# arpitbansal297/Cold-Diffusion-Models

Hardware: NVIDIA H100
Metric: training-step images/sec (CelebA-128 deblur UNet, config 3) (higher is better)
Workload: dtype tf32

## Files before the change

### cold_diffusion_models_b200/csrc/conv_tc.cu

```cuda
#include "tc_common.cuh"
#include "conv_epilogue.cuh"

namespace {

constexpr int kTileM = 128;
constexpr int kChunkK = 32;
constexpr int kABytes = kTileM * 128;
constexpr int kThreads = 288;
constexpr int kConsumerWarps = 8;

struct TcParams {
  int B, Hg, Wg;
  int TW, TH, TN;
  int tiles_x, tiles_y, tiles_n, tiles_co, total_tiles;
  int sy, sx;
  int Cout;
  int nsrc;
  int ntaps[2];
  int kchunks[2];
  int wpb[2];
  int8_t dy[2][CD_MAX_TAPS];
  int8_t dx[2][CD_MAX_TAPS];
  float* out; int out_ld; int Ho, Wo; int oys, oxs, oy0, ox0;
  const float* bias;
  const float* resid; int resid_ld;
  int act; int round_tf32;
  float* out2; int out2_ld;
  const float* aux; int aux_ld;
  int nbox[2];
  int8_t boxdx[2][3];
  int8_t boxend[2][3];
  int8_t taporder[2][CD_MAX_TAPS];
  int tapoff[2][CD_MAX_TAPS];
};

__device__ __forceinline__ long long tile_pixel(const TcParams& p, int tile, int m) {
  int mt = tile / p.tiles_co;
  const int tx = mt % p.tiles_x; mt /= p.tiles_x;
  const int ty = mt % p.tiles_y;
  const int tn = mt / p.tiles_y;
  const int gx = tx * p.TW + m % p.TW, gy = ty * p.TH + (m / p.TW) % p.TH, b = tn * p.TN + m / (p.TW * p.TH);
  if (b >= p.B) return -1;
  return (static_cast<long long>(b) * p.Ho + (gy * p.oys + p.oy0)) * p.Wo + (gx * p.oxs + p.ox0);
}

__device__ __forceinline__ void epi_pair(const TcParams& p, long long pix, int col, float v0, float v1) {
  if (col + 1 < p.Cout) {
    float2 v = make_float2(v0, v1);
    if (p.bias) { const float2 b = __ldg(reinterpret_cast<const float2*>(p.bias + col)); v.x += b.x; v.y += b.y; }
    if (p.resid) { const float2 r = *reinterpret_cast<const float2*>(p.resid + pix * p.resid_ld + col); v.x += r.x; v.y += r.y; }
    if (p.out2) *reinterpret_cast<float2*>(p.out2 + pix * p.out2_ld + col) = v;
    if (p.act == CD_ACT_GELU) { v.x = cd_gelu(v.x); v.y = cd_gelu(v.y); }
    else if (p.act == CD_ACT_GELU_BWD) {
      const float2 a = *reinterpret_cast<const float2*>(p.aux + pix * p.aux_ld + col);
      v.x *= cd_gelu_grad(a.x); v.y *= cd_gelu_grad(a.y);
    }
    if (p.round_tf32) { v.x = cd_round_tf32(v.x); v.y = cd_round_tf32(v.y); }
    *reinterpret_cast<float2*>(p.out + pix * p.out_ld + col) = v;
  } else if (col < p.Cout) {
    float v = v0;
    if (p.bias) v += p.bias[col];
    if (p.resid) v += p.resid[pix * p.resid_ld + col];
    if (p.out2) p.out2[pix * p.out2_ld + col] = v;
    if (p.act == CD_ACT_GELU) v = cd_gelu(v);
    else if (p.act == CD_ACT_GELU_BWD) v *= cd_gelu_grad(p.aux[pix * p.aux_ld + col]);
    if (p.round_tf32) v = cd_round_tf32(v);
    p.out[pix * p.out_ld + col] = v;
  }
}

template <int BN, int STAGES, bool STG = false, bool F16 = false, int CTAS = 1, bool PAIR = false>
__global__ void __launch_bounds__(kThreads, CTAS)
conv_tc_kernel(const __grid_constant__ CUtensorMap mapA0, const __grid_constant__ CUtensorMap mapA1,
               const __grid_constant__ CUtensorMap mapB0, const __grid_constant__ CUtensorMap mapB1,
               const TcParams p) {
  constexpr int kBBytes = BN * 128;
  constexpr int kStageBytes = kABytes + kBBytes;
  constexpr int kChunkElems = F16 ? 64 : kChunkK;

  extern __shared__ uint8_t smem_raw[];
  const uint32_t raw_addr = smem_u32(smem_raw);
  const uint32_t pad = (1024u - (raw_addr & 1023u)) & 1023u;
  uint8_t* smem = smem_raw + pad;
  uint64_t* bars = reinterpret_cast<uint64_t*>(smem + STAGES * kStageBytes);
  uint64_t* full_bar = bars;
  uint64_t* empty_bar = bars + STAGES;
  static_assert(2 * STAGES * 8 <= 256, "barrier block is 256 bytes");
  float* epi_stage = reinterpret_cast<float*>(smem + STAGES * kStageBytes + 256);

  const int warp = threadIdx.x >> 5;
  const int lane = threadIdx.x & 31;
  const int wg = threadIdx.x >> 7;

  if (threadIdx.x == 0) {
    for (int i = 0; i < STAGES; ++i) { mbar_init(&full_bar[i], 1); mbar_init(&empty_bar[i], kConsumerWarps * (PAIR ? 2 : 1)); }
    asm volatile("fence.mbarrier_init.release.cluster;" ::: "memory");
  }
  if constexpr (PAIR) cluster_sync(); else __syncthreads();
  const uint32_t rank = PAIR ? cluster_ctarank() : 0;
  const int unit0 = PAIR ? blockIdx.x / 2 : blockIdx.x, ustride = PAIR ? gridDim.x / 2 : gridDim.x;
  const int units = PAIR ? p.tiles_co * ((p.total_tiles / p.tiles_co + 1) / 2) : p.total_tiles;
  auto tile_of = [&](int u) { return PAIR ? ((u / p.tiles_co) * 2 + static_cast<int>(rank)) * p.tiles_co + u % p.tiles_co : u; };

  const int kiters = p.ntaps[0] * p.kchunks[0] + (p.nsrc > 1 ? p.ntaps[1] * p.kchunks[1] : 0);

  if (warp == kConsumerWarps) {
    if (elect_one()) {
      uint32_t stage = 0, ph = 0;
      for (int u = unit0; u < units; u += ustride) {
        const int tile = tile_of(u);
        const int co_t = tile % p.tiles_co;
        int mt = tile / p.tiles_co;
        const int tx = mt % p.tiles_x; mt /= p.tiles_x;
        const int ty = mt % p.tiles_y;
        const int tn = mt / p.tiles_y;
        const int x0 = tx * p.TW * p.sx, y0 = ty * p.TH * p.sy, n0 = tn * p.TN, co0 = co_t * BN;
        for (int s = 0; s < p.nsrc; ++s) {
          const CUtensorMap* mA = s ? &mapA1 : &mapA0;
          const CUtensorMap* mB = s ? &mapB1 : &mapB0;
          const int wbase = p.wpb[s] ? n0 * p.ntaps[s] : 0;
          for (int tap = 0; tap < p.ntaps[s]; ++tap) {
            const int xin = x0 + p.dx[s][tap], yin = y0 + p.dy[s][tap];
            for (int kc = 0; kc < p.kchunks[s]; ++kc) {
              mbar_wait(&empty_bar[stage], ph ^ 1u);
              mbar_expect_tx(&full_bar[stage], kStageBytes);
              const uint32_t sa = smem_u32(smem + stage * kStageBytes);
              tma_load_4d(sa, mA, &full_bar[stage], kc * kChunkElems, xin, yin, n0);
              if constexpr (PAIR)
                tma_load_3d_mc(sa + kABytes + rank * (kBBytes / 2), mB, &full_bar[stage], kc * kChunkElems, co0 + static_cast<int>(rank) * (BN / 2),
                               wbase + tap, static_cast<uint16_t>(3));
              else
                tma_load_3d(sa + kABytes, mB, &full_bar[stage], kc * kChunkElems, co0, wbase + tap);
              if (++stage == STAGES) { stage = 0; ph ^= 1u; }
            }
          }
        }
      }
    }
    __syncwarp();
  } else {
    const int cw = wg;
    const int tid = threadIdx.x & 127;
    const int rl = (tid >> 5) * 16 + (lane >> 2);
    const int q2 = (lane & 3) * 2;
    float acc[BN / 2];
    uint32_t stage = 0, ph = 0;
    auto release = [&](uint32_t st) {
      __syncwarp();
      if (lane == 0) { mbar_arrive(&empty_bar[st]); if constexpr (PAIR) mbar_arrive_cluster(&empty_bar[st], rank ^ 1u); }
    };
    for (int u = unit0; u < units; u += ustride) {
      const int tile = tile_of(u);
      uint32_t prev = 0;
      for (int k = 0; k < kiters; ++k) {
        mbar_wait(&full_bar[stage], ph);
        wgmma_fence();
        const uint32_t sa = smem_u32(smem + stage * kStageBytes);
        const uint64_t da = make_kmajor_sw128_desc(sa + cw * (kABytes / 2));
        const uint64_t db = make_kmajor_sw128_desc(sa + kABytes);
#pragma unroll
        for (int kk = 0; kk < 4; ++kk) {
          if constexpr (F16) wgmma_f16<BN>(acc, da + uint64_t(kk * 2), db + uint64_t(kk * 2), (k | kk) != 0 ? 1u : 0u);
          else wgmma_tf32<BN>(acc, da + uint64_t(kk * 2), db + uint64_t(kk * 2), (k | kk) != 0 ? 1u : 0u);
        }
        wgmma_commit();
        wgmma_wait<1>();
        if (k > 0) release(prev);
        prev = stage;
        if (++stage == STAGES) { stage = 0; ph ^= 1u; }
      }
      wgmma_wait<0>();
      if (kiters > 0) release(prev);

      const int co0 = (tile % p.tiles_co) * BN;
      const long long pix0 = tile_pixel(p, tile, cw * 64 + rl);
      const long long pix1 = tile_pixel(p, tile, cw * 64 + rl + 8);
      if constexpr (STG) {
        float* st = epi_stage + cw * 64 * kEpiStageStride;
        const int bar_id = 1 + cw;
#pragma unroll
        for (int c = 0; c < BN; c += 32) {
          if (co0 + c + 32 <= p.Cout) {
            asm volatile("bar.sync %0, 128;" :: "r"(bar_id) : "memory");
#pragma unroll
            for (int j = c / 8; j < c / 8 + 4; ++j) {
              *reinterpret_cast<float2*>(st + rl * kEpiStageStride + 8 * j - c + q2) = make_float2(acc[4 * j], acc[4 * j + 1]);
              *reinterpret_cast<float2*>(st + (rl + 8) * kEpiStageStride + 8 * j - c + q2) = make_float2(acc[4 * j + 2], acc[4 * j + 3]);
            }
            asm volatile("bar.sync %0, 128;" :: "r"(bar_id) : "memory");
            const int w4 = tid >> 5;
            if (w4 < 2) {
              const int row = w4 * 32 + lane;
              uint32_t r[32];
#pragma unroll
              for (int e = 0; e < 32; ++e) r[e] = __float_as_uint(st[row * kEpiStageStride + e]);
              const long long pix = tile_pixel(p, tile, cw * 64 + row);
              cd_epilogue_staged32(r, st + w4 * 32 * kEpiStageStride, lane, pix < 0 ? 0 : pix, pix >= 0, co0 + c, p);
            }
          } else {
#pragma unroll
            for (int j = c / 8; j < c / 8 + 4; ++j) {
              if (pix0 >= 0) epi_pair(p, pix0, co0 + 8 * j + q2, acc[4 * j], acc[4 * j + 1]);
              if (pix1 >= 0) epi_pair(p, pix1, co0 + 8 * j + q2, acc[4 * j + 2], acc[4 * j + 3]);
            }
          }
        }
      } else {
#pragma unroll
        for (int j = 0; j < BN / 8; ++j) {
          if (pix0 >= 0) epi_pair(p, pix0, co0 + 8 * j + q2, acc[4 * j], acc[4 * j + 1]);
          if (pix1 >= 0) epi_pair(p, pix1, co0 + 8 * j + q2, acc[4 * j + 2], acc[4 * j + 3]);
        }
      }
    }
  }
  if constexpr (PAIR) cluster_sync();
}

constexpr int kRowsTW = 16, kRowsTH = kTileM / kRowsTW;
constexpr int kRowsBoxBytes = kRowsTW * (kRowsTH + 2) * 128;

template <int BN, int TH, int ABOXES, int STAGES>
__device__ __forceinline__ void rows_producer(const CUtensorMap& mapA0, const CUtensorMap& mapA1, const CUtensorMap& mapB0,
                                              const CUtensorMap& mapB1, const TcParams& p, uint8_t* abox, uint8_t* wtile,
                                              uint64_t* afull, uint64_t* aempty, uint64_t* full_bar, uint64_t* empty_bar) {
  constexpr int kBBytes = BN * 128;
  constexpr int kBoxBytes = kRowsTW * (TH + 2) * 128;
  if (elect_one()) {
    uint32_t stage = 0, ph = 0, ai = 0, aph = 0;
    for (int tile = blockIdx.x; tile < p.total_tiles; tile += gridDim.x) {
      const int co0 = (tile % p.tiles_co) * BN;
      int mt = tile / p.tiles_co;
      const int x0 = (mt % p.tiles_x) * kRowsTW; mt /= p.tiles_x;
      const int y0 = (mt % p.tiles_y) * TH;
      const int n = mt / p.tiles_y;
      for (int s = 0; s < p.nsrc; ++s) {
        const CUtensorMap* mA = s ? &mapA1 : &mapA0;
        const CUtensorMap* mB = s ? &mapB1 : &mapB0;
        for (int kc = 0; kc < p.kchunks[s]; ++kc) {
          for (int b = 0, i = 0; b < p.nbox[s]; ++b) {
            mbar_wait(&aempty[ai], aph ^ 1u);
            mbar_expect_tx(&afull[ai], kBoxBytes);
            tma_load_4d(smem_u32(abox + ai * kBoxBytes), mA, &afull[ai], kc * kChunkK, x0 + p.boxdx[s][b], y0 - 1, n);
            if (++ai == ABOXES) { ai = 0; aph ^= 1u; }
            for (; i < p.boxend[s][b]; ++i) {
              mbar_wait(&empty_bar[stage], ph ^ 1u);
              mbar_expect_tx(&full_bar[stage], kBBytes);
              tma_load_3d(smem_u32(wtile + stage * kBBytes), mB, &full_bar[stage], kc * kChunkK, co0, p.taporder[s][i]);
              if (++stage == STAGES) { stage = 0; ph ^= 1u; }
            }
          }
        }
      }
    }
  }
  __syncwarp();
}

template <int BN, int ABOXES, int STAGES, int CTAS>
__global__ void __launch_bounds__(kThreads, CTAS)
conv_rows_kernel(const __grid_constant__ CUtensorMap mapA0, const __grid_constant__ CUtensorMap mapA1,
                 const __grid_constant__ CUtensorMap mapB0, const __grid_constant__ CUtensorMap mapB1, const __grid_constant__ TcParams p) {
  constexpr int kBBytes = BN * 128;
  extern __shared__ uint8_t smem_raw[];
  const uint32_t raw_addr = smem_u32(smem_raw);
  uint8_t* smem = smem_raw + ((1024u - (raw_addr & 1023u)) & 1023u);
  uint8_t* abox = smem;
  uint8_t* wtile = smem + ABOXES * kRowsBoxBytes;
  uint64_t* bars = reinterpret_cast<uint64_t*>(wtile + STAGES * kBBytes);
  uint64_t* full_bar = bars;
  uint64_t* empty_bar = bars + STAGES;
  uint64_t* afull = bars + 2 * STAGES;
  uint64_t* aempty = bars + 2 * STAGES + ABOXES;
  static_assert(2 * (STAGES + ABOXES) * 8 <= 256, "barrier block is 256 bytes");
  const int warp = threadIdx.x >> 5, lane = threadIdx.x & 31, wg = threadIdx.x >> 7;
  if (threadIdx.x == 0) {
    for (int i = 0; i < STAGES; ++i) { mbar_init(&full_bar[i], 1); mbar_init(&empty_bar[i], kConsumerWarps); }
    for (int i = 0; i < ABOXES; ++i) { mbar_init(&afull[i], 1); mbar_init(&aempty[i], kConsumerWarps); }
    asm volatile("fence.mbarrier_init.release.cluster;" ::: "memory");
  }
  __syncthreads();

  if (warp == kConsumerWarps) {
    rows_producer<BN, kRowsTH, ABOXES, STAGES>(mapA0, mapA1, mapB0, mapB1, p, abox, wtile, afull, aempty, full_bar, empty_bar);
    return;
  }

  const int tid = threadIdx.x & 127;
  const int rl = (tid >> 5) * 16 + (lane >> 2);
  const int q2 = (lane & 3) * 2;
  auto release = [&](uint64_t* bar) { __syncwarp(); if (lane == 0) mbar_arrive(bar); };
  float acc[BN / 2];
  uint32_t stage = 0, ph = 0, ai = 0, aph = 0;
  for (int tile = blockIdx.x; tile < p.total_tiles; tile += gridDim.x) {
    int k = 0;
    uint32_t prev = 0, prev_a = 0;
    for (int s = 0; s < p.nsrc; ++s) {
      for (int kc = 0; kc < p.kchunks[s]; ++kc) {
        for (int b = 0, i = 0; b < p.nbox[s]; ++b) {
          mbar_wait(&afull[ai], aph);
          const uint32_t abase = smem_u32(abox + ai * kRowsBoxBytes) + wg * (kABytes / 2);
          for (const int i0 = i; i < p.boxend[s][b]; ++i, ++k) {
            mbar_wait(&full_bar[stage], ph);
            wgmma_fence();
            const uint64_t da = make_kmajor_sw128_desc(abase + p.tapoff[s][i]);
            const uint64_t db = make_kmajor_sw128_desc(smem_u32(wtile + stage * kBBytes));
#pragma unroll
            for (int kk = 0; kk < 4; ++kk)
              wgmma_tf32<BN>(acc, da + uint64_t(kk * 2), db + uint64_t(kk * 2), (k | kk) != 0 ? 1u : 0u);
            wgmma_commit();
            wgmma_wait<1>();
            if (k > 0) release(&empty_bar[prev]);
            if (k > 0 && i == i0) release(&aempty[prev_a]);
            prev = stage;
            if (++stage == STAGES) { stage = 0; ph ^= 1u; }
          }
          prev_a = ai;
          if (++ai == ABOXES) { ai = 0; aph ^= 1u; }
        }
      }
    }
    wgmma_wait<0>();
    if (k > 0) { release(&empty_bar[prev]); release(&aempty[prev_a]); }

    const int co0 = (tile % p.tiles_co) * BN;
    int mt = tile / p.tiles_co;
    const int x0 = (mt % p.tiles_x) * kRowsTW; mt /= p.tiles_x;
    const int y0 = (mt % p.tiles_y) * kRowsTH;
    const int n = mt / p.tiles_y;
#pragma unroll
    for (int h = 0; h < 2; ++h) {
      const int m = wg * 64 + rl + 8 * h;
      const int gx = x0 + m % kRowsTW, gy = y0 + m / kRowsTW;
      if (gx >= p.Wg || gy >= p.Hg) continue;
      const long long pix = (static_cast<long long>(n) * p.Ho + (gy * p.oys + p.oy0)) * p.Wo + (gx * p.oxs + p.ox0);
#pragma unroll
      for (int j = 0; j < BN / 8; ++j) epi_pair(p, pix, co0 + 8 * j + q2, acc[4 * j + 2 * h], acc[4 * j + 2 * h + 1]);
    }
  }
}

constexpr int kR256TH = 16;
constexpr int kR256BoxBytes = kRowsTW * (kR256TH + 2) * 128;
constexpr int kR256Slice = 128 * 128;
constexpr int kR256Threads = 384;
constexpr int kR256RegsLow = 40, kR256RegsHigh = 232;

constexpr int kOpFull = 0, kOpEmpty = 2, kBiasFull = 4, kBiasEmpty = 5, kEpiBars = 6;

__host__ __device__ __forceinline__ const float* rows256_operand(const TcParams& p) {
  return p.resid ? p.resid : (p.act == CD_ACT_GELU_BWD ? p.aux : nullptr);
}

template <int BN>
__device__ __forceinline__ void rows256_epilogue_producer(const CUtensorMap& mapE, const TcParams& p, int cw, uint8_t* so2,
                                                          float* sbias, uint64_t* eb) {
  const int lane = threadIdx.x & 31;
  const bool opnd = rows256_operand(p) != nullptr;
  uint32_t bph = 0, oph = 0;
  for (int tile = blockIdx.x; tile < p.total_tiles; tile += gridDim.x) {
    const int co0 = (tile % p.tiles_co) * BN;
    int mt = tile / p.tiles_co;
    const int x0 = (mt % p.tiles_x) * kRowsTW; mt /= p.tiles_x;
    const int yw = (mt % p.tiles_y) * kR256TH + 8 * cw;
    const int n = mt / p.tiles_y;
    if (yw >= p.Hg) continue;
    if (p.bias) {
      mbar_wait(&eb[kBiasEmpty], bph ^ 1u);
      for (int i = lane; i < BN; i += 32) sbias[i] = co0 + i < p.Cout ? p.bias[co0 + i] : 0.f;
      mbar_arrive(&eb[kBiasFull]);
      bph ^= 1u;
    }
    if (opnd && lane == 0) {
      for (int c = 0; c < BN / 32 && co0 + 32 * c < p.Cout; ++c)
        for (int h = 0; h < 2; ++h) {
          mbar_wait(&eb[kOpEmpty + h], ((oph >> h) & 1u) ^ 1u);
          mbar_expect_tx(&eb[kOpFull + h], kR256Slice / 2);
          tma_load_4d(smem_u32(so2 + h * (kR256Slice / 2)), &mapE, &eb[kOpFull + h], co0 + 32 * c, x0, yw + 4 * h, n);
          oph ^= 1u << h;
        }
    }
    __syncwarp();
  }
}

template <int BN, int ABOXES, int STAGES>
__global__ void __launch_bounds__(kR256Threads, 1)
conv_rows256_kernel(const __grid_constant__ CUtensorMap mapA0, const __grid_constant__ CUtensorMap mapA1,
                    const __grid_constant__ CUtensorMap mapB0, const __grid_constant__ CUtensorMap mapB1,
                    const __grid_constant__ CUtensorMap mapO, const __grid_constant__ CUtensorMap mapO2,
                    const __grid_constant__ CUtensorMap mapE, const __grid_constant__ TcParams p) {
  constexpr int kBBytes = BN * 128;
  extern __shared__ uint8_t smem_raw[];
  const uint32_t raw_addr = smem_u32(smem_raw);
  uint8_t* smem = smem_raw + ((1024u - (raw_addr & 1023u)) & 1023u);
  uint8_t* abox = smem;
  uint8_t* wtile = smem + ABOXES * kR256BoxBytes;
  uint8_t* stg = wtile + STAGES * kBBytes;
  uint64_t* bars = reinterpret_cast<uint64_t*>(stg + 4 * kR256Slice);
  uint64_t* full_bar = bars;
  uint64_t* empty_bar = bars + STAGES;
  uint64_t* afull = bars + 2 * STAGES;
  uint64_t* aempty = bars + 2 * STAGES + ABOXES;
  uint64_t* ebars = bars + 2 * (STAGES + ABOXES);
  float* sbias = reinterpret_cast<float*>(bars + 32);
  static_assert(2 * (STAGES + ABOXES) * 8 + 2 * kEpiBars * 8 <= 256, "barrier block is 256 bytes");
  const int warp = threadIdx.x >> 5, lane = threadIdx.x & 31, wg = threadIdx.x >> 7;
  if (threadIdx.x == 0) {
    for (int i = 0; i < STAGES; ++i) { mbar_init(&full_bar[i], 1); mbar_init(&empty_bar[i], kConsumerWarps); }
    for (int i = 0; i < ABOXES; ++i) { mbar_init(&afull[i], 1); mbar_init(&aempty[i], kConsumerWarps); }
    for (int w = 0; w < 2; ++w) {
      uint64_t* eb = ebars + w * kEpiBars;
      for (int h = 0; h < 2; ++h) { mbar_init(&eb[kOpFull + h], 1); mbar_init(&eb[kOpEmpty + h], kConsumerWarps / 2); }
      mbar_init(&eb[kBiasFull], 32);
      mbar_init(&eb[kBiasEmpty], kConsumerWarps / 2);
    }
    asm volatile("fence.mbarrier_init.release.cluster;" ::: "memory");
  }
  __syncthreads();

  if (wg == 0) {
    asm volatile("setmaxnreg.dec.sync.aligned.u32 %0;" :: "n"(kR256RegsLow));
    if (warp == 0)
      rows_producer<BN, kR256TH, ABOXES, STAGES>(mapA0, mapA1, mapB0, mapB1, p, abox, wtile, afull, aempty, full_bar, empty_bar);
    else if (warp <= 2 && (p.bias || rows256_operand(p)))
      rows256_epilogue_producer<BN>(mapE, p, warp - 1, stg + (warp - 1) * 2 * kR256Slice + kR256Slice, sbias + (warp - 1) * BN,
                                    ebars + (warp - 1) * kEpiBars);
    return;
  }
  asm volatile("setmaxnreg.inc.sync.aligned.u32 %0;" :: "n"(kR256RegsHigh));

  const int cw = wg - 1;
  const int tid = threadIdx.x & 127;
  const int rl = (tid >> 5) * 16 + (lane >> 2);
  const int q2 = (lane & 3) * 2;
  const bool storer = tid == 0;
  uint8_t* so = stg + cw * 2 * kR256Slice;
  uint8_t* so2 = so + kR256Slice;
  uint64_t* eb = ebars + cw * kEpiBars;
  const float* sb = sbias + cw * BN;
  const bool opnd = rows256_operand(p) != nullptr;
  auto release = [&](uint64_t* bar) { __syncwarp(); if (lane == 0) mbar_arrive(bar); };
  auto wg_sync = [&]() { asm volatile("bar.sync %0, 128;" :: "r"(1 + cw) : "memory"); };
  float acc[2][BN / 2];
  uint32_t stage = 0, ph = 0, ai = 0, aph = 0;
  uint32_t bph = 0, oph = 0;
  bool held = false;
  for (int tile = blockIdx.x; tile < p.total_tiles; tile += gridDim.x) {
    int k = 0;
    uint32_t prev = 0, prev_a = 0;
    for (int s = 0; s < p.nsrc; ++s) {
      for (int kc = 0; kc < p.kchunks[s]; ++kc) {
        for (int b = 0, i = 0; b < p.nbox[s]; ++b) {
          mbar_wait(&afull[ai], aph);
          const uint32_t abase = smem_u32(abox + ai * kR256BoxBytes) + cw * kABytes;
          for (const int i0 = i; i < p.boxend[s][b]; ++i, ++k) {
            mbar_wait(&full_bar[stage], ph);
            wgmma_fence();
            const uint64_t da0 = make_kmajor_sw128_desc(abase + p.tapoff[s][i]);
            const uint64_t da1 = make_kmajor_sw128_desc(abase + p.tapoff[s][i] + kABytes / 2);
            const uint64_t db = make_kmajor_sw128_desc(smem_u32(wtile + stage * kBBytes));
#pragma unroll
            for (int kk = 0; kk < 4; ++kk) {
              wgmma_tf32<BN>(acc[0], da0 + uint64_t(kk * 2), db + uint64_t(kk * 2), (k | kk) != 0 ? 1u : 0u);
              wgmma_tf32<BN>(acc[1], da1 + uint64_t(kk * 2), db + uint64_t(kk * 2), (k | kk) != 0 ? 1u : 0u);
            }
            wgmma_commit();
            wgmma_wait<1>();
            if (k > 0) release(&empty_bar[prev]);
            if (k > 0 && i == i0) release(&aempty[prev_a]);
            prev = stage;
            if (++stage == STAGES) { stage = 0; ph ^= 1u; }
          }
          prev_a = ai;
          if (++ai == ABOXES) { ai = 0; aph ^= 1u; }
        }
      }
    }
    wgmma_wait<0>();
    if (k > 0) { release(&empty_bar[prev]); release(&aempty[prev_a]); }

    const int co0 = (tile % p.tiles_co) * BN;
    int mt = tile / p.tiles_co;
    const int x0 = (mt % p.tiles_x) * kRowsTW; mt /= p.tiles_x;
    const int yw = (mt % p.tiles_y) * kR256TH + 8 * cw;
    const int n = mt / p.tiles_y;
    if (yw >= p.Hg) continue;
    if (p.bias) { mbar_wait(&eb[kBiasFull], bph); bph ^= 1u; }
#pragma unroll
    for (int c = 0; c < BN / 32; ++c) {
      if (co0 + 32 * c >= p.Cout) break;
      if (storer) bulk_wait_read<0>();
      wg_sync();
      if (held) { release(&eb[kOpEmpty]); release(&eb[kOpEmpty + 1]); held = false; }
#pragma unroll
      for (int h = 0; h < 2; ++h) {
        auto soff = [&](int e, int jj) {
          const int rr = 64 * h + rl + 8 * e;
          return rr * 128 + ((((8 * jj + q2) >> 2) ^ (rr & 7)) << 4) + (q2 & 3) * 4;
        };
        float2 o[2][4];
        if (opnd) {
          mbar_wait(&eb[kOpFull + h], (oph >> h) & 1u);
          oph ^= 1u << h;
#pragma unroll
          for (int e = 0; e < 2; ++e)
#pragma unroll
            for (int jj = 0; jj < 4; ++jj) o[e][jj] = *reinterpret_cast<const float2*>(so2 + soff(e, jj));
        }
        float2 v[2][4];
#pragma unroll
        for (int e = 0; e < 2; ++e)
#pragma unroll
          for (int jj = 0; jj < 4; ++jj) v[e][jj] = make_float2(acc[h][16 * c + 4 * jj + 2 * e], acc[h][16 * c + 4 * jj + 2 * e + 1]);
        if (p.bias) {
#pragma unroll
          for (int jj = 0; jj < 4; ++jj) {
            const float2 b = *reinterpret_cast<const float2*>(sb + 32 * c + 8 * jj + q2);
#pragma unroll
            for (int e = 0; e < 2; ++e) { v[e][jj].x += b.x; v[e][jj].y += b.y; }
          }
        }
        if (p.resid) {
#pragma unroll
          for (int e = 0; e < 2; ++e)
#pragma unroll
            for (int jj = 0; jj < 4; ++jj) { v[e][jj].x += o[e][jj].x; v[e][jj].y += o[e][jj].y; }
        }
        if (p.out2) {
#pragma unroll
          for (int e = 0; e < 2; ++e)
#pragma unroll
            for (int jj = 0; jj < 4; ++jj) *reinterpret_cast<float2*>(so2 + soff(e, jj)) = v[e][jj];
        }
        if (p.act == CD_ACT_GELU) {
#pragma unroll
          for (int e = 0; e < 2; ++e)
#pragma unroll
            for (int jj = 0; jj < 4; ++jj) { v[e][jj].x = cd_gelu(v[e][jj].x); v[e][jj].y = cd_gelu(v[e][jj].y); }
        } else if (p.act == CD_ACT_GELU_BWD) {
#pragma unroll
          for (int e = 0; e < 2; ++e)
#pragma unroll
            for (int jj = 0; jj < 4; ++jj) { v[e][jj].x *= cd_gelu_grad(o[e][jj].x); v[e][jj].y *= cd_gelu_grad(o[e][jj].y); }
        }
        if (p.round_tf32) {
#pragma unroll
          for (int e = 0; e < 2; ++e)
#pragma unroll
            for (int jj = 0; jj < 4; ++jj) { v[e][jj].x = cd_round_tf32(v[e][jj].x); v[e][jj].y = cd_round_tf32(v[e][jj].y); }
        }
#pragma unroll
        for (int e = 0; e < 2; ++e)
#pragma unroll
          for (int jj = 0; jj < 4; ++jj) *reinterpret_cast<float2*>(so + soff(e, jj)) = v[e][jj];
        if (opnd && !p.out2) release(&eb[kOpEmpty + h]);
      }
      fence_proxy_async();
      wg_sync();
      if (storer) {
        tma_store_4d(&mapO, smem_u32(so), co0 + 32 * c, x0, yw, n);
        if (p.out2) tma_store_4d(&mapO2, smem_u32(so2), co0 + 32 * c, x0, yw, n);
        bulk_commit();
      }
      held = opnd && p.out2;
    }
    if (p.bias) release(&eb[kBiasEmpty]);
  }
  if (storer) bulk_wait<0>();
}


int g_tf32_map_dtype = 1;

template <auto Kernel, size_t kSmem, int CTAS, bool PAIR = false>
int launch_persistent(const CUtensorMap* maps, const TcParams& p, cudaStream_t st) {
  static_assert(kSmem <= 232448, "dynamic shared memory of one CTA (227 KB)");
  static_assert(CTAS == 1 || 2 * (kSmem + 1024) <= 233472, "two CTAs per SM must fit the 228 KB of shared memory");
  CD_CUDA(smem_limit_once<Kernel>(kSmem));
  if constexpr (PAIR) {
    const int units = p.tiles_co * ((p.total_tiles / p.tiles_co + 1) / 2), slots = cd_num_sms() / 2;
    cudaLaunchConfig_t cfg = {};
    cudaLaunchAttribute attr[1];
    attr[0].id = cudaLaunchAttributeClusterDimension;
    attr[0].val.clusterDim.x = 2; attr[0].val.clusterDim.y = 1; attr[0].val.clusterDim.z = 1;
    cfg.gridDim = dim3(2 * (units < slots ? units : slots)); cfg.blockDim = dim3(kThreads);
    cfg.dynamicSmemBytes = kSmem; cfg.stream = st; cfg.attrs = attr; cfg.numAttrs = 1;
    CD_CUDA(cudaLaunchKernelEx(&cfg, Kernel, maps[0], maps[1], maps[2], maps[3], p));
  } else {
    const int slots = cd_num_sms() * CTAS;
    const int grid = p.total_tiles < slots ? p.total_tiles : slots;
    Kernel<<<grid, kThreads, kSmem, st>>>(maps[0], maps[1], maps[2], maps[3], p);
  }
  CD_LAUNCH_CHECK();
  return 0;
}

template <int BN, int STAGES, bool STG = false, bool F16 = false, int CTAS = 1, bool PAIR = false>
int launch(const CUtensorMap* maps, const TcParams& p, cudaStream_t st) {
  constexpr size_t smem = size_t(STAGES) * (kABytes + BN * 128) + 1024 + 256 + (STG ? sizeof(float) * 2 * 64 * kEpiStageStride : 0);
  return launch_persistent<conv_tc_kernel<BN, STAGES, STG, F16, CTAS, PAIR>, smem, CTAS, PAIR>(maps, p, st);
}

template <int BN, int ABOXES, int STAGES, int CTAS = 1>
int launch_rows(const CUtensorMap* maps, const TcParams& p, cudaStream_t st) {
  constexpr size_t smem = size_t(ABOXES) * kRowsBoxBytes + size_t(STAGES) * BN * 128 + 1024 + 256;
  return launch_persistent<conv_rows_kernel<BN, ABOXES, STAGES, CTAS>, smem, CTAS>(maps, p, st);
}

template <int BN, int ABOXES, int STAGES>
int launch_rows256(const CUtensorMap* maps, const TcParams& p, cudaStream_t st) {
  constexpr size_t smem = size_t(ABOXES) * kR256BoxBytes + size_t(STAGES) * BN * 128 + 4 * kR256Slice + 256 + 2 * BN * 4 + 1024;
  static_assert(smem <= 232448, "dynamic shared memory of one CTA (227 KB)");
  constexpr auto kernel = conv_rows256_kernel<BN, ABOXES, STAGES>;
  CD_CUDA(smem_limit_once<kernel>(smem));
  const int sms = cd_num_sms();
  const int grid = p.total_tiles < sms ? p.total_tiles : sms;
  kernel<<<grid, kR256Threads, smem, st>>>(maps[0], maps[1], maps[2], maps[3], maps[4], maps[5], maps[6], p);
  CD_LAUNCH_CHECK();
  return 0;
}

bool operands_ok(const CdConvDesc* d, int chunk_elems, int esz, bool report) {
#define TC_CHECK(cond, ...) do { if (!(cond)) { if (report) cd_set_error(__VA_ARGS__); return false; } } while (0)
  TC_CHECK(d->nsrc >= 1 && d->nsrc <= 2, "conv_tc: nsrc must be 1 or 2");
  TC_CHECK(d->act != CD_ACT_GELU_BWD || (d->aux && (reinterpret_cast<uintptr_t>(d->aux) & 15) == 0 && d->aux_ld % 4 == 0), "conv_tc: GELU_BWD needs an aligned aux");
  TC_CHECK((reinterpret_cast<uintptr_t>(d->out) & 15) == 0 && d->out_ld % 4 == 0, "conv_tc: out must be 16B aligned");
  TC_CHECK(!d->resid || ((reinterpret_cast<uintptr_t>(d->resid) & 15) == 0 && d->resid_ld % 4 == 0), "conv_tc: resid alignment");
  TC_CHECK(!d->out2 || ((reinterpret_cast<uintptr_t>(d->out2) & 15) == 0 && d->out2_ld % 4 == 0), "conv_tc: out2 alignment");
  TC_CHECK(!d->bias || (reinterpret_cast<uintptr_t>(d->bias) & 15) == 0, "conv_tc: bias alignment");
  for (int s = 0; s < d->nsrc; ++s) {
    const CdConvSrc& cs = d->s[s];
    TC_CHECK(cs.C % chunk_elems == 0 && cs.C > 0, "conv_tc: source channels %d not a multiple of %d", cs.C, chunk_elems);
    TC_CHECK(cs.ntaps >= 1 && cs.ntaps <= CD_MAX_TAPS, "conv_tc: bad ntaps");
    TC_CHECK((reinterpret_cast<uintptr_t>(cs.src) & 15) == 0 && (cs.ld * esz) % 16 == 0, "conv_tc: src must be 16B aligned");
    TC_CHECK((reinterpret_cast<uintptr_t>(cs.w) & 15) == 0, "conv_tc: weights must be 16B aligned");
  }
#undef TC_CHECK
  return true;
}

TcParams desc_params(const CdConvDesc* d, int chunk_elems) {
  TcParams p{};
  p.B = d->B; p.Hg = d->Hg; p.Wg = d->Wg; p.sy = d->sy; p.sx = d->sx; p.Cout = d->Cout; p.nsrc = d->nsrc;
  for (int s = 0; s < 2; ++s) {
    const CdConvSrc& cs = d->s[s < d->nsrc ? s : 0];
    p.ntaps[s] = cs.ntaps; p.kchunks[s] = cs.C / chunk_elems; p.wpb[s] = cs.w_per_batch;
    for (int t = 0; t < cs.ntaps; ++t) { p.dy[s][t] = (int8_t)cs.dy[t]; p.dx[s][t] = (int8_t)cs.dx[t]; }
  }
  p.out = d->out; p.out_ld = d->out_ld; p.Ho = d->Ho; p.Wo = d->Wo;
  p.oys = d->oys; p.oxs = d->oxs; p.oy0 = d->oy0; p.ox0 = d->ox0;
  p.bias = d->bias; p.resid = d->resid; p.resid_ld = d->resid_ld; p.act = d->act; p.round_tf32 = d->round_tf32;
  p.out2 = d->out2; p.out2_ld = d->out2_ld; p.aux = d->aux; p.aux_ld = d->aux_ld;
  return p;
}

}

extern "C" int cd_conv_tc_set_tf32_maps(int enable) { g_tf32_map_dtype = enable ? 1 : 0; return 0; }

static int g_use_2cta = 0;
extern "C" int cd_conv_tc_set_2cta(int mode) { g_use_2cta = mode; return 0; }
static int g_2cta_bn = 0;
extern "C" int cd_conv_tc_set_2cta_bn(int mask) { g_2cta_bn = mask & (128 | 64); return 0; }
static int g_use_halo = 0;
extern "C" int cd_conv_tc_set_halo(int enable) { g_use_halo = enable; return 0; }
static int g_ctas2 = 128 | 64;
extern "C" int cd_conv_tc_set_two_ctas(int mask) { g_ctas2 = mask & (128 | 64); return 0; }
static int g_epi_staged = 0;
constexpr int kStagedMaxKIters = 16;
constexpr int kStagedMidKIters = 48;
extern "C" int cd_conv_tc_set_staged_epilogue(int mode) { g_epi_staged = mode; return 0; }

static double tc_cost(long long m_tiles, int Cout, int BN, int sms, bool pair = false) {
  if (pair) {
    const long long tiles = ((m_tiles + 1) / 2) * (Cout / 256), slots = sms / 2;
    return double((tiles + slots - 1) / slots) * 256.0;
  }
  const long long tiles = m_tiles * ((Cout + BN - 1) / BN);
  const double rate = BN == 256 ? 0.92 : (BN == 128 ? 0.75 : 0.40);
  return double((tiles + sms - 1) / sms) * BN / rate;
}

static int conv_fwd_tc_impl(const CdConvDesc* d, cudaStream_t st, bool f16);
int cd_conv_fwd_tc(const CdConvDesc* d, cudaStream_t st) { return conv_fwd_tc_impl(d, st, false); }

extern "C" int cd_conv_fwd_f16_probe(const CdConvDesc* d, void* stream) {
  CD_REQUIRE(d != nullptr && d->nsrc >= 1 && d->nsrc <= 2, "cd_conv_fwd_f16_probe: bad descriptor");
  return conv_fwd_tc_impl(d, static_cast<cudaStream_t>(stream), true);
}

static int conv_fwd_rows(const CdConvDesc* d, cudaStream_t st, int mode);

static int conv_fwd_tc_impl(const CdConvDesc* d, cudaStream_t st, bool f16) {
  if (!f16 && g_epi_staged == 0) {
    if ((g_use_halo == 0 && !g_use_2cta) || g_use_halo == 1 || g_use_halo == 2 || g_use_halo == 4 || g_use_halo == 6) {
      const int r = conv_fwd_rows(d, st, g_use_halo);
      if (r <= 0) return r;
    }
  }
  const CUtensorMapDataType dt = f16 ? CU_TENSOR_MAP_DATA_TYPE_FLOAT16 : (g_tf32_map_dtype ? CU_TENSOR_MAP_DATA_TYPE_TFLOAT32 : CU_TENSOR_MAP_DATA_TYPE_FLOAT32);
  const int esz = map_elem_bytes(dt), chunk_elems = 128 / esz;
  if (!operands_ok(d, chunk_elems, esz, true)) return -1;
  TcParams p = desc_params(d, chunk_elems);
  if (d->Wg >= 128) {
    CD_REQUIRE(d->Wg % 128 == 0, "conv_tc: Wg >= 128 must be a multiple of 128 (got %d)", d->Wg);
    p.TW = 128; p.TH = 1; p.TN = 1;
  } else {
    CD_REQUIRE(is_pow2(d->Wg), "conv_tc: Wg < 128 must be a power of two (got %d)", d->Wg);
    p.TW = d->Wg;
    int th = 128 / p.TW;
    if (th > d->Hg) th = d->Hg;
    CD_REQUIRE(is_pow2(th) && d->Hg % th == 0, "conv_tc: unsupported Hg %d for Wg %d", d->Hg, d->Wg);
    p.TH = th; p.TN = 128 / (p.TW * p.TH);
  }
  CD_REQUIRE(p.TW * d->sx <= 256 && p.TH * d->sy <= 256, "conv_tc: strided box too large");
  p.tiles_x = d->Wg / p.TW; p.tiles_y = d->Hg / p.TH; p.tiles_n = cd_cdiv(d->B, p.TN);
  int BN = (d->Cout % 256 == 0) ? 256 : (d->Cout > 64 ? 128 : 64);
  int kiters_host = 0;
  for (int s = 0; s < d->nsrc; ++s) kiters_host += d->s[s].ntaps * (d->s[s].C / chunk_elems);
  const bool staged = !f16 &&
                      ( g_epi_staged == 2 || (g_epi_staged == 1 && kiters_host <= kStagedMaxKIters) ||
                      (g_epi_staged == 3 && kiters_host <= kStagedMidKIters));
  bool pair = false;
  const long long mt = static_cast<long long>(p.tiles_x) * p.tiles_y * p.tiles_n;
  const int sms = cd_num_sms();
  if (BN == 256) {
    double best = tc_cost(mt, d->Cout, 256, sms);
    if (tc_cost(mt, d->Cout, 128, sms) < best) { BN = 128; best = tc_cost(mt, d->Cout, 128, sms); }
    if (!f16 && !staged && g_use_2cta && mt >= 2 && (g_use_2cta == 2 || tc_cost(mt, d->Cout, 256, sms, true) < best)) {
      BN = 256; pair = true;
    }
  } else if (!f16 && !staged && g_use_2cta && (g_2cta_bn & BN) && d->Cout % BN == 0 && (g_use_2cta == 2 || mt >= 2 * sms)) {
    pair = true;
  }
  p.tiles_co = cd_cdiv(d->Cout, BN);
  p.total_tiles = p.tiles_x * p.tiles_y * p.tiles_n * p.tiles_co;

  CUtensorMap maps[4];
  for (int s = 0; s < 2; ++s) {
    const CdConvSrc& cs = d->s[s < d->nsrc ? s : 0];
    CD_REQUIRE(!cs.w_per_batch || p.TN == 1, "conv_tc: per-batch weights need >=128 pixels per image");
    if (!encode_nhwc(&maps[s], dt, cs.src, cs.ld, cs.C, cs.W, cs.H, d->B, 1, 1, 0, 0, p.TW * d->sx, p.TH * d->sy, p.TN, d->sx, d->sy,
                     s ? "A1" : "A0") ||
        !encode_weights(&maps[2 + s], dt, cs.w, cs.C, d->Cout, cs.ntaps * (cs.w_per_batch ? d->B : 1), pair ? BN / 2 : BN,
                        s ? "B1" : "B0"))
      return -1;
  }
  if (f16) {
    if (BN == 256) return launch<256, 4, false, true>(maps, p, st);
    if (BN == 128) return launch<128, 6, false, true>(maps, p, st);
    return launch<64, 8, false, true>(maps, p, st);
  }
  if (staged) {
    if (BN == 256) return launch<256, 3, true>(maps, p, st);
    if (BN == 128) return launch<128, 4, true>(maps, p, st);
    return launch<64, 6, true>(maps, p, st);
  }
  if (pair) {
    if (BN == 256) return launch<256, 4, false, false, 1, true>(maps, p, st);
    if (BN == 128) return launch<128, 6, false, false, 1, true>(maps, p, st);
    return launch<64, 8, false, false, 1, true>(maps, p, st);
  }
  const int ctas2 = p.total_tiles > sms ? g_ctas2 : 0;
  if (BN == 256) return launch<256, 4>(maps, p, st);
  if (BN == 128) return (ctas2 & 128) ? launch<128, 3, false, false, 2>(maps, p, st) : launch<128, 6>(maps, p, st);
  return (ctas2 & 64) ? launch<64, 4, false, false, 2>(maps, p, st) : launch<64, 8>(maps, p, st);
}

static int conv_fwd_rows(const CdConvDesc* d, cudaStream_t st, int mode) {
  const bool by_shape = mode == 0;
  if (d->sy != 1 || d->sx != 1 || !operands_ok(d, kChunkK, 4, false)) return 1;
  for (int s = 0; s < d->nsrc; ++s) {
    const CdConvSrc& cs = d->s[s];
    if (cs.w_per_batch || cs.W != d->Wg || cs.H != d->Hg) return 1;
    for (int t = 0; t < cs.ntaps; ++t) if (cs.dy[t] < -1 || cs.dy[t] > 1 || cs.dx[t] < -1 || cs.dx[t] > 1) return 1;
  }
  TcParams p = desc_params(d, kChunkK);
  p.TW = kRowsTW; p.TH = kRowsTH; p.TN = 1;
  p.tiles_x = cd_cdiv(d->Wg, kRowsTW); p.tiles_y = cd_cdiv(d->Hg, kRowsTH); p.tiles_n = d->B;
  const int BN = d->Cout > 64 ? 128 : 64;
  p.tiles_co = cd_cdiv(d->Cout, BN);
  p.total_tiles = p.tiles_x * p.tiles_y * p.tiles_n * p.tiles_co;
  const int sms = cd_num_sms();
  if (by_shape && p.total_tiles <= sms) return 1;
  const int tiles256 = p.tiles_x * cd_cdiv(d->Hg, kR256TH) * p.tiles_n * p.tiles_co;
  const bool rows256 = (mode == 4 || (by_shape && 4 * tiles256 >= 3 * sms)) && d->oys == 1 && d->oxs == 1 && d->oy0 == 0 &&
                       d->ox0 == 0 && d->Ho == d->Hg && d->Wo == d->Wg && !(d->resid && d->act == CD_ACT_GELU_BWD) &&
                       d->Cout % 4 == 0;
  if (rows256) { p.TH = kR256TH; p.tiles_y = cd_cdiv(d->Hg, kR256TH); p.total_tiles = tiles256; }
  const CUtensorMapDataType dt = g_tf32_map_dtype ? CU_TENSOR_MAP_DATA_TYPE_TFLOAT32 : CU_TENSOR_MAP_DATA_TYPE_FLOAT32;
  CUtensorMap maps[7] = {};
  for (int s = 0; s < 2; ++s) {
    const CdConvSrc& cs = d->s[s < d->nsrc ? s : 0];
    int i = 0;
    for (int dx = -1; dx <= 1; ++dx) {
      const int i0 = i;
      for (int t = 0; t < cs.ntaps; ++t)
        if (cs.dx[t] == dx) { p.taporder[s][i] = (int8_t)t; p.tapoff[s][i] = (cs.dy[t] + 1) * kRowsTW * 128; ++i; }
      if (i > i0) { p.boxdx[s][p.nbox[s]] = (int8_t)dx; p.boxend[s][p.nbox[s]] = (int8_t)i; ++p.nbox[s]; }
    }
    if (s == 0 && cs.ntaps < 3 * p.nbox[0]) return 1;
    if (!encode_nhwc(&maps[s], dt, cs.src, cs.ld, cs.C, cs.W, cs.H, d->B, 1, 1, 0, 0, kRowsTW, p.TH + 2, 1, 1, 1,
                     s ? "rows A1" : "rows A0") ||
        !encode_weights(&maps[2 + s], dt, cs.w, cs.C, d->Cout, cs.ntaps, BN, s ? "rows B1" : "rows B0"))
      return -1;
  }
  if (rows256) {
    const float* o2 = d->out2 ? d->out2 : d->out;
    const int o2ld = d->out2 ? d->out2_ld : d->out_ld;
    if (!encode_nhwc(&maps[4], CU_TENSOR_MAP_DATA_TYPE_FLOAT32, d->out, d->out_ld, d->Cout, d->Wg, d->Hg, d->B, 1, 1, 0, 0, kRowsTW,
                     kR256TH / 2, 1, 1, 1, "rows out") ||
        !encode_nhwc(&maps[5], CU_TENSOR_MAP_DATA_TYPE_FLOAT32, o2, o2ld, d->Cout, d->Wg, d->Hg, d->B, 1, 1, 0, 0, kRowsTW,
                     kR256TH / 2, 1, 1, 1, "rows out2"))
      return -1;
    const float* opnd = rows256_operand(p);
    const int opnd_ld = d->resid ? d->resid_ld : d->aux_ld;
    if (opnd && !encode_nhwc(&maps[6], CU_TENSOR_MAP_DATA_TYPE_FLOAT32, opnd, opnd_ld, d->Cout, d->Wg, d->Hg, d->B, 1, 1, 0, 0,
                             kRowsTW, kR256TH / 4, 1, 1, 1, "rows operand"))
      return -1;
    if (BN == 128) return launch_rows256<128, 3, 3>(maps, p, st);
    return launch_rows256<64, 3, 6>(maps, p, st);
  }
  const int ctas2 = p.total_tiles > sms ? g_ctas2 : 0;
  if (BN == 128) return (ctas2 & 128) ? launch_rows<128, 3, 3, 2>(maps, p, st) : launch_rows<128, 6, 4>(maps, p, st);
  return (ctas2 & 64) ? launch_rows<64, 3, 6, 2>(maps, p, st) : launch_rows<64, 6, 8>(maps, p, st);
}
```

Before: 706.5.

## Add weights-on-M rows256 conv kernel using register-sourced wgmma for 64-channel outputs

Adds a rows256 convolution kernel variant that puts the 64 output channels on the wgmma M side, loading weight fragments from shared memory into registers (RS wgmma) and streaming the pixel boxes as the B descriptor, with double-buffered fragment loads. It is selected by default (by_shape) for BN=64 layers with Cout divisible by 32, and via a new halo mode 5. This transposes the MMA orientation to make better use of the 128-row M dimension when Cout is small, at the cost of extra register pressure and shared-memory fragment loads per k-step.

```diff
diff --git a/cold_diffusion_models_b200/csrc/conv_tc.cu b/cold_diffusion_models_b200/csrc/conv_tc.cu
--- a/cold_diffusion_models_b200/csrc/conv_tc.cu
+++ b/cold_diffusion_models_b200/csrc/conv_tc.cu
@@ -570,6 +570,205 @@
   if (storer) bulk_wait<0>();
 }
 
+template <int ABOXES, int STAGES>
+__global__ void __launch_bounds__(kR256Threads, 1)
+conv_rows256_wm_kernel(const __grid_constant__ CUtensorMap mapA0, const __grid_constant__ CUtensorMap mapA1,
+                       const __grid_constant__ CUtensorMap mapB0, const __grid_constant__ CUtensorMap mapB1,
+                       const __grid_constant__ CUtensorMap mapO, const __grid_constant__ CUtensorMap mapO2,
+                       const __grid_constant__ CUtensorMap mapE, const __grid_constant__ TcParams p) {
+  constexpr int BN = 64;
+  constexpr int kBBytes = BN * 128;
+  extern __shared__ uint8_t smem_raw[];
+  const uint32_t raw_addr = smem_u32(smem_raw);
+  uint8_t* smem = smem_raw + ((1024u - (raw_addr & 1023u)) & 1023u);
+  uint8_t* abox = smem;
+  uint8_t* wtile = smem + ABOXES * kR256BoxBytes;
+  uint8_t* stg = wtile + STAGES * kBBytes;
+  uint64_t* bars = reinterpret_cast<uint64_t*>(stg + 4 * kR256Slice);
+  uint64_t* full_bar = bars;
+  uint64_t* empty_bar = bars + STAGES;
+  uint64_t* afull = bars + 2 * STAGES;
+  uint64_t* aempty = bars + 2 * STAGES + ABOXES;
+  uint64_t* ebars = bars + 2 * (STAGES + ABOXES);
+  float* sbias = reinterpret_cast<float*>(bars + 32);
+  static_assert(2 * (STAGES + ABOXES) * 8 + 2 * kEpiBars * 8 <= 256, "barrier block is 256 bytes");
+  const int warp = threadIdx.x >> 5, lane = threadIdx.x & 31, wg = threadIdx.x >> 7;
+  if (threadIdx.x == 0) {
+    for (int i = 0; i < STAGES; ++i) { mbar_init(&full_bar[i], 1); mbar_init(&empty_bar[i], kConsumerWarps); }
+    for (int i = 0; i < ABOXES; ++i) { mbar_init(&afull[i], 1); mbar_init(&aempty[i], kConsumerWarps); }
+    for (int w = 0; w < 2; ++w) {
+      uint64_t* eb = ebars + w * kEpiBars;
+      for (int h = 0; h < 2; ++h) { mbar_init(&eb[kOpFull + h], 1); mbar_init(&eb[kOpEmpty + h], kConsumerWarps / 2); }
+      mbar_init(&eb[kBiasFull], 32);
+      mbar_init(&eb[kBiasEmpty], kConsumerWarps / 2);
+    }
+    asm volatile("fence.mbarrier_init.release.cluster;" ::: "memory");
+  }
+  __syncthreads();
+
+  if (wg == 0) {
+    asm volatile("setmaxnreg.dec.sync.aligned.u32 %0;" :: "n"(kR256RegsLow));
+    if (warp == 0)
+      rows_producer<BN, kR256TH, ABOXES, STAGES>(mapA0, mapA1, mapB0, mapB1, p, abox, wtile, afull, aempty, full_bar, empty_bar);
+    else if (warp <= 2 && (p.bias || rows256_operand(p)))
+      rows256_epilogue_producer<BN>(mapE, p, warp - 1, stg + (warp - 1) * 2 * kR256Slice + kR256Slice, sbias + (warp - 1) * BN,
+                                    ebars + (warp - 1) * kEpiBars);
+    return;
+  }
+  asm volatile("setmaxnreg.inc.sync.aligned.u32 %0;" :: "n"(kR256RegsHigh));
+
+  const int cw = wg - 1;
+  const int tid = threadIdx.x & 127;
+  const int g = lane >> 2, t = lane & 3;
+  const int ch = 8 * (tid >> 5) + g;
+  const int wrow = ch * 128 + 4 * t;
+  const bool storer = tid == 0;
+  uint8_t* so = stg + cw * 2 * kR256Slice;
+  uint8_t* so2 = so + kR256Slice;
+  uint64_t* eb = ebars + cw * kEpiBars;
+  const float* sb = sbias + cw * BN;
+  const bool opnd = rows256_operand(p) != nullptr;
+  auto release = [&](uint64_t* bar) { __syncwarp(); if (lane == 0) mbar_arrive(bar); };
+  auto wg_sync = [&]() { asm volatile("bar.sync %0, 128;" :: "r"(1 + cw) : "memory"); };
+  auto load_frags = [&](uint32_t (&f)[4][4], uint32_t st) {
+    const uint8_t* wt = wtile + st * kBBytes + wrow;
+#pragma unroll
+    for (int kk = 0; kk < 4; ++kk) {
+      const int c0 = ((2 * kk) ^ g) << 4, c1 = ((2 * kk + 1) ^ g) << 4;
+      f[kk][0] = *reinterpret_cast<const uint32_t*>(wt + c0);
+      f[kk][1] = *reinterpret_cast<const uint32_t*>(wt + 32 * 128 + c0);
+      f[kk][2] = *reinterpret_cast<const uint32_t*>(wt + c1);
+      f[kk][3] = *reinterpret_cast<const uint32_t*>(wt + 32 * 128 + c1);
+    }
+  };
+  const int kiters = p.kchunks[0] * p.ntaps[0] + (p.nsrc > 1 ? p.kchunks[1] * p.ntaps[1] : 0);
+  float acc[BN];
+  uint32_t fa[4][4], fb[4][4];
+  uint32_t stage = 0, ph = 0, ai = 0, aph = 0;
+  uint32_t bph = 0, oph = 0;
+  bool held = false;
+  for (int tile = blockIdx.x; tile < p.total_tiles; tile += gridDim.x) {
+    int k = 0;
+    uint32_t prev = 0, prev_a = 0;
+    if (kiters > 0) { mbar_wait(&full_bar[stage], ph); load_frags(fa, stage); }
+    for (int s = 0; s < p.nsrc; ++s) {
+      for (int kc = 0; kc < p.kchunks[s]; ++kc) {
+        for (int b = 0, i = 0; b < p.nbox[s]; ++b) {
+          mbar_wait(&afull[ai], aph);
+          const uint32_t abase = smem_u32(abox + ai * kR256BoxBytes) + cw * kABytes;
+          for (const int i0 = i; i < p.boxend[s][b]; ++i, ++k) {
+            const uint32_t nstage = stage + 1 == STAGES ? 0 : stage + 1, nph = stage + 1 == STAGES ? ph ^ 1u : ph;
+            const uint64_t db = make_kmajor_sw128_desc(abase + p.tapoff[s][i]);
+            auto step = [&](uint32_t (&cur)[4][4], uint32_t (&nxt)[4][4]) {
+              wgmma_fence();
+#pragma unroll
+              for (int kk = 0; kk < 4; ++kk) wgmma_tf32_rs<128>(acc, cur[kk], db + uint64_t(kk * 2), (k | kk) != 0 ? 1u : 0u);
+              wgmma_commit();
+              wgmma_wait<1>();
+              if (k > 0) release(&empty_bar[prev]);
+              if (k > 0 && i == i0) release(&aempty[prev_a]);
+              if (k + 1 < kiters) { mbar_wait(&full_bar[nstage], nph); load_frags(nxt, nstage); }
+            };
+            if (k & 1) step(fb, fa); else step(fa, fb);
+            prev = stage; stage = nstage; ph = nph;
+          }
+          prev_a = ai;
+          if (++ai == ABOXES) { ai = 0; aph ^= 1u; }
+        }
+      }
+    }
+    wgmma_wait<0>();
+    if (k > 0) { release(&empty_bar[prev]); release(&aempty[prev_a]); }
+
+    const int co0 = (tile % p.tiles_co) * BN;
+    int mt = tile / p.tiles_co;
+    const int x0 = (mt % p.tiles_x) * kRowsTW; mt /= p.tiles_x;
+    const int yw = (mt % p.tiles_y) * kR256TH + 8 * cw;
+    const int n = mt / p.tiles_y;
+    if (yw >= p.Hg) continue;
+    if (p.bias) { mbar_wait(&eb[kBiasFull], bph); bph ^= 1u; }
+#pragma unroll
+    for (int c = 0; c < BN / 32; ++c) {
+      if (co0 + 32 * c >= p.Cout) break;
+      if (storer) bulk_wait_read<0>();
+      wg_sync();
+      if (held) { release(&eb[kOpEmpty]); release(&eb[kOpEmpty + 1]); held = false; }
+      const float bv = p.bias ? sb[32 * c + ch] : 0.f;
+#pragma unroll
+      for (int h = 0; h < 2; ++h) {
+        float v[8][2];
+#pragma unroll
+        for (int jj = 0; jj < 8; ++jj)
+#pragma unroll
+          for (int e = 0; e < 2; ++e) v[jj][e] = acc[4 * (8 * h + jj) + 2 * c + e];
+        if (p.bias) {
+#pragma unroll
+          for (int jj = 0; jj < 8; ++jj)
+#pragma unroll
+            for (int e = 0; e < 2; ++e) v[jj][e] += bv;
+        }
+        auto soff = [&](int jj, int e) {
+          const int r = 64 * h + 8 * jj + 2 * t + e;
+          return r * 128 + (((ch >> 2) ^ (2 * t + e)) << 4) + (ch & 3) * 4;
+        };
+        float o[8][2];
+        if (opnd) {
+          mbar_wait(&eb[kOpFull + h], (oph >> h) & 1u);
+          oph ^= 1u << h;
+#pragma unroll
+          for (int jj = 0; jj < 8; ++jj)
+#pragma unroll
+            for (int e = 0; e < 2; ++e) o[jj][e] = *reinterpret_cast<const float*>(so2 + soff(jj, e));
+        }
+        if (p.resid) {
+#pragma unroll
+          for (int jj = 0; jj < 8; ++jj)
+#pragma unroll
+            for (int e = 0; e < 2; ++e) v[jj][e] += o[jj][e];
+        }
+        if (p.out2) {
+#pragma unroll
+          for (int jj = 0; jj < 8; ++jj)
+#pragma unroll
+            for (int e = 0; e < 2; ++e) *reinterpret_cast<float*>(so2 + soff(jj, e)) = v[jj][e];
+        }
+        if (p.act == CD_ACT_GELU) {
+#pragma unroll
+          for (int jj = 0; jj < 8; ++jj)
+#pragma unroll
+            for (int e = 0; e < 2; ++e) v[jj][e] = cd_gelu(v[jj][e]);
+        } else if (p.act == CD_ACT_GELU_BWD) {
+#pragma unroll
+          for (int jj = 0; jj < 8; ++jj)
+#pragma unroll
+            for (int e = 0; e < 2; ++e) v[jj][e] *= cd_gelu_grad(o[jj][e]);
+        }
+        if (p.round_tf32) {
+#pragma unroll
+          for (int jj = 0; jj < 8; ++jj)
+#pragma unroll
+            for (int e = 0; e < 2; ++e) v[jj][e] = cd_round_tf32(v[jj][e]);
+        }
+#pragma unroll
+        for (int jj = 0; jj < 8; ++jj)
+#pragma unroll
+          for (int e = 0; e < 2; ++e) *reinterpret_cast<float*>(so + soff(jj, e)) = v[jj][e];
+        if (opnd && !p.out2) release(&eb[kOpEmpty + h]);
+      }
+      fence_proxy_async();
+      wg_sync();
+      if (storer) {
+        tma_store_4d(&mapO, smem_u32(so), co0 + 32 * c, x0, yw, n);
+        if (p.out2) tma_store_4d(&mapO2, smem_u32(so2), co0 + 32 * c, x0, yw, n);
+        bulk_commit();
+      }
+      held = opnd && p.out2;
+    }
+    if (p.bias) release(&eb[kBiasEmpty]);
+  }
+  if (storer) bulk_wait<0>();
+}
+
 
 int g_tf32_map_dtype = 1;
 
@@ -608,11 +807,14 @@
   return launch_persistent<conv_rows_kernel<BN, ABOXES, STAGES, CTAS>, smem, CTAS>(maps, p, st);
 }
 
-template <int BN, int ABOXES, int STAGES>
+template <int BN, int ABOXES, int STAGES, bool WM = false>
 int launch_rows256(const CUtensorMap* maps, const TcParams& p, cudaStream_t st) {
+  static_assert(!WM || BN == 64, "the weights-on-M kernel has 64 output channels per tile");
   constexpr size_t smem = size_t(ABOXES) * kR256BoxBytes + size_t(STAGES) * BN * 128 + 4 * kR256Slice + 256 + 2 * BN * 4 + 1024;
   static_assert(smem <= 232448, "dynamic shared memory of one CTA (227 KB)");
-  constexpr auto kernel = conv_rows256_kernel<BN, ABOXES, STAGES>;
+  constexpr auto kernel = [] {
+    if constexpr (WM) return conv_rows256_wm_kernel<ABOXES, STAGES>; else return conv_rows256_kernel<BN, ABOXES, STAGES>;
+  }();
   CD_CUDA(smem_limit_once<kernel>(smem));
   const int sms = cd_num_sms();
   const int grid = p.total_tiles < sms ? p.total_tiles : sms;
@@ -694,7 +896,7 @@
 
 static int conv_fwd_tc_impl(const CdConvDesc* d, cudaStream_t st, bool f16) {
   if (!f16 && g_epi_staged == 0) {
-    if ((g_use_halo == 0 && !g_use_2cta) || g_use_halo == 1 || g_use_halo == 2 || g_use_halo == 4 || g_use_halo == 6) {
+    if ((g_use_halo == 0 && !g_use_2cta) || g_use_halo == 1 || g_use_halo == 2 || g_use_halo == 4 || g_use_halo == 5 || g_use_halo == 6) {
       const int r = conv_fwd_rows(d, st, g_use_halo);
       if (r <= 0) return r;
     }
@@ -785,7 +987,7 @@
   const int sms = cd_num_sms();
   if (by_shape && p.total_tiles <= sms) return 1;
   const int tiles256 = p.tiles_x * cd_cdiv(d->Hg, kR256TH) * p.tiles_n * p.tiles_co;
-  const bool rows256 = (mode == 4 || (by_shape && 4 * tiles256 >= 3 * sms)) && d->oys == 1 && d->oxs == 1 && d->oy0 == 0 &&
+  const bool rows256 = (mode == 4 || mode == 5 || (by_shape && 4 * tiles256 >= 3 * sms)) && d->oys == 1 && d->oxs == 1 && d->oy0 == 0 &&
                        d->ox0 == 0 && d->Ho == d->Hg && d->Wo == d->Wg && !(d->resid && d->act == CD_ACT_GELU_BWD) &&
                        d->Cout % 4 == 0;
   if (rows256) { p.TH = kR256TH; p.tiles_y = cd_cdiv(d->Hg, kR256TH); p.total_tiles = tiles256; }
@@ -820,6 +1022,7 @@
                              kRowsTW, kR256TH / 4, 1, 1, 1, "rows operand"))
       return -1;
     if (BN == 128) return launch_rows256<128, 3, 3>(maps, p, st);
+    if ((mode == 5 || by_shape) && d->Cout % 32 == 0) return launch_rows256<64, 3, 6, true>(maps, p, st);
     return launch_rows256<64, 3, 6>(maps, p, st);
   }
   const int ctas2 = p.total_tiles > sms ? g_ctas2 : 0;
```

New measurement: 703.5, median of 6. Within noise of the previous version (-0.4%).
